# IvanPopov/video-flow-ml

Measured on AMD Instinct MI355X. Metric: flow-fields/sec @1080p seq5 MOF_sintel, higher is better.
Workload: dtype mixed (per-layer MFMA count, f32 accumulate): {"corr": 1, "update_block.encoder.convf1": 1, "update_block.encoder.convf2": 1, "update_block.gru.convq1.iter": "2a", "update_block.gru.convzr1.iter": 1, "update_block.gru.convzr2.iter": 1, "update_block.mask.0": 1, "update_block.mask.2": 1, "update_bloc

## Files before the change

### include/vfml.h

```cpp
#ifndef VFML_H
#define VFML_H
#include <stddef.h>
#include <stdint.h>

#ifdef __cplusplus
extern "C" {
#endif

#define VFML_ABI_VERSION 26

enum {
  VFML_EPI_NONE = 0,
  VFML_EPI_RELU = 1,
  VFML_EPI_TANH = 2,
  VFML_EPI_SIGMOID = 3,
  VFML_EPI_TANH_RELU = 4,
  VFML_EPI_GRU_ZR = 5,
  VFML_EPI_GRU_Q = 6,
  VFML_EPI_ADD_AUX = 7,
};

enum { VFML_FMT_F32 = 0, VFML_FMT_S16 = 1,
       VFML_FMT_F16 = 2 };

// ... 70 lines not shown
int vfml_instnorm_stats(const float* x, int n, int hw, int c, float eps,
                        float* stats, void* workspace, void* stream);
int vfml_instnorm_apply(const float* x, const float* stats, const float* res,
                        const float* res_stats, int n, int hw, int c, float* out, int out_fmt, void* stream);

int vfml_avgpool2x2(const float* x, int n, int h, int w, int c, float* out, void* stream);

int vfml_corr_lookup(const float* const* pyr, const int32_t* hl, const int32_t* wl,
                     const int32_t* ld, int levels, int radius, int nmaps, int q_per_map,
                     const float* coords, int ld_coords, float* out, int ld_out, int out_fmt, int vol_fmt, int vol_tile,
                     void* stream);
#define VFML_VOL_F16_LEVELS(m) (0x100 | (m))

int vfml_corr_lookup_indirect(const float* const* table, const int32_t* hl, const int32_t* wl, const int32_t* ld,
                              int levels, int radius, int nmaps, int q_per_map, const float* coords, int ld_coords,
                              float* out, int ld_out, int out_fmt, int vol_fmt, int vol_tile, void* stream);
int vfml_corr_lookup_indirect_bidir(const float* const* table, const int32_t* hl, const int32_t* wl, const int32_t* ld,
                                    int levels, int radius, int nmaps, int q_per_map, const float* coords, int ld_coords,
                                    int dir_coords, float* out, int ld_out, int dir_out, int dir_tab, int out_fmt, int vol_fmt,
                                    int vol_tile, void* stream);
int vfml_ptr_table_set(void* table, const void* const* ptrs, int n, void* stream);

#define VFML_SEED_NONE 0
#define VFML_SEED_LOAD 1
#define VFML_SEED_STORE 2
int vfml_window_seed(const void* cells, int ncentres, int rows, int cols, float* state, int ld_state, int h_off, int mf_off,
                     int ld_ctx, void* stream);

int vfml_flow_rows7(const float* flow, int n, int h, int w, float* rows, void* stream);

int vfml_conv3x3_c64(const float* in, int ld_in, int n, int h, int w, const void* w_hi, const void* w_lo, int kp, float w_scale,
                     const float* bias, float* out, int ldo, double* stats_part, void* stream);

int vfml_flow_half(const float* flow, int n, int h, int w, const void* w1_hi, int kp1, float w1_scale, const float* b1,
                   const void* w2_hi, int kp2, float w2_scale, const float* b2, float* out, int ld_out, void* stream);

int vfml_tapsum3x3(const float* t, int ld_t, const float* bias, int n, int h, int w, float* out, int parts, int64_t part_stride,
                   void* stream);
int vfml_tapsum3x3_update(const float* t, int ld_t, const float* bias, int n, int h, int w, int parts, int64_t part_stride,
                          float* coords1, float* flow_a, int ld_a, float* flow_b, int ld_b, int fmt_b, void* stream);

int vfml_coords_update(float* coords1, const float* delta, int n, int h, int w,
                       float* flow_a, int ld_a, float* flow_b, int ld_b, int fmt_b, void* stream);
int vfml_coords_init(float* coords1, int n, int h, int w, void* stream);

int vfml_convex_upsample(const float* coords1, int ch, const float* mask, int ld_mask,
                         int h, int w, float* out, void* stream);

int64_t vfml_instnorm_finalize_workspace_bytes(int chunks, int c);
int vfml_instnorm_finalize(const double* part, int n, int chunks, int c, int hw, float eps, float* stats,
                           void* workspace, int64_t workspace_bytes, void* stream);

int vfml_stem7x7s2_chunks(int h, int w);
int vfml_stem7x7s2(const float* frames, int n, int h, int w, const void* w_hi, const void* w_lo, float w_scale,
                   const float* bias, float* out, double* stats_part, void* stream);

int vfml_flow_lod(const float* flow, int h, int w, float* out, void* stream);

enum { VFML_ENCODE_GAMEDEV = 0, VFML_ENCODE_RG8 = 1, VFML_ENCODE_RGB8 = 2 };
int vfml_flow_encode(const float* flow, int h, int w, int mode, float width, float height, float scale,
                     float clamp, float two_clamp, unsigned char* out, void* stream);

enum { VFML_TAA_SIMPLE = 0, VFML_TAA_BILINEAR = 1, VFML_TAA_BILATERAL = 2 };
enum { VFML_PIX_U8 = 0, VFML_PIX_F32 = 1, VFML_PIX_F64 = 2 };
int vfml_taa_blend(const void* current, int cur_type, const float* flow, const void* history, int hist_type,
                   void* out, int out_type, int h, int w, int mode, double alpha, double sigma_color, void* stream);
// ... 102 lines not shown
```

### video-flow-ml_amd/vfml/hip.py

```python
import ctypes
import os
import subprocess
from ctypes import POINTER, c_char_p, c_double, c_float, c_int, c_int32, c_int64, c_void_p

import torch

_HERE = os.path.dirname(os.path.abspath(__file__))
LIB_PATH = os.environ.get("VFML_LIB") or os.path.join(_HERE, "libvfml_hip.so")
CSRC = os.path.join(_HERE, "csrc")
SOURCES = ["api.hip", "conv_gemm.hip", "conv_gemm_split.hip", "conv_gemm_tapx.hip", "conv_split_plan.hip", "stem.hip", "flow_half.hip", "enc_conv.hip", "norm_pool.hip", "flow_ops.hip", "effects.hip", "correct.hip", "render.hip", "text.hip", "turbulence.hip", "resize.hip", "jpeg.hip", "jpeg_decode.hip", "jpeg_decode_sync.hip", "deflate.hip", "attention.hip", "dwconv.hip"]

STATS_ROWS_F32, STATS_ROWS_S16 = 128, 32
EPI_NONE, EPI_RELU, EPI_TANH, EPI_SIGMOID, EPI_TANH_RELU, EPI_GRU_ZR, EPI_GRU_Q, EPI_ADD_AUX = range(8)
FMT_F32, FMT_S16, FMT_F16 = 0, 1, 2


def vol_f16_levels(mask):
    return 0x100 | mask


def _vol_mask(vol_fmt, levels):
    return (15 if vol_fmt == FMT_F16 else (vol_fmt & 15 if vol_fmt & 0x100 else 0)) & ((1 << levels) - 1)

KORDER_TAP, KORDER_CBLOCK, KORDER_CBLOCK64 = 0, 1, 2
CONV_SWAP_CROSS, CONV_MFMA2, CONV_MFMA1, CONV_MFMA2A, CONV_PER_TAP = 1, 2, 4, 8, 16


class ConvDesc(ctypes.Structure):
    _fields_ = [
        ("in0", c_void_p), ("c0", c_int32), ("ld0", c_int32),
        ("in1", c_void_p), ("c1", c_int32), ("ld1", c_int32),
        ("n", c_int32), ("h", c_int32), ("w", c_int32),
        ("weight", c_void_p), ("bias", c_void_p),
        ("cout", c_int32), ("kh", c_int32), ("kw", c_int32), ("stride", c_int32),
        ("pad_h", c_int32), ("pad_w", c_int32),
        ("out", c_void_p), ("ldo", c_int32),
        ("epilogue", c_int32), ("split", c_int32), ("out_scale", c_float),
        ("aux0", c_void_p), ("ld_aux0", c_int32),
        ("aux1", c_void_p), ("ld_aux1", c_int32),
        ("addend", c_void_p), ("ld_addend", c_int32),
        ("out_t", c_void_p), ("ld_out_t", c_int32),
        ("flags", c_int32),
        ("stats_part", c_void_p),
        ("ksplit_ws", c_void_p),
        ("proj_hi", c_void_p), ("proj_lo", c_void_p), ("proj_n", c_int32), ("proj_kp", c_int32), ("proj_scale", c_float),
        ("proj_out", c_void_p), ("ld_proj", c_int32),
        ("addend_ind", c_void_p),
    ]


COMMON_FLAGS = ["-fno-slp-vectorize"]
EXTRA_FLAGS = {}


def build(force=False, verbose=False):
    srcs = [os.path.join(CSRC, s) for s in SOURCES]
    hdrs = [os.path.join(CSRC, "vfml_common.h"), os.path.join(CSRC, "conv_split_common.h"),
# ... 54 lines not shown
    L.vfml_instnorm_workspace_bytes.argtypes = [c_int, c_int, c_int]
    L.vfml_instnorm_stats.argtypes = [c_void_p, c_int, c_int, c_int, c_float, c_void_p, c_void_p, c_void_p]
    L.vfml_softmax_rows_f16.argtypes = [c_void_p, c_int64, c_int, c_int64, c_void_p, c_int64, c_float, c_void_p]
    L.vfml_attention_plane_workspace_bytes.restype = c_int64
    L.vfml_attention_plane_workspace_bytes.argtypes = [c_int]
    L.vfml_attention_plane_f16.argtypes = [c_void_p, c_int64, c_void_p, c_int64, c_int, c_int, c_float, c_float, c_void_p, c_int64,
                                           c_void_p, c_void_p]
    L.vfml_dwconv2d.argtypes = [c_void_p, c_int64, c_int, c_int, c_int, c_int, c_int, c_void_p, c_void_p, c_void_p, c_int64, c_int, c_int,
                                c_int, c_void_p]
    L.vfml_gelu_rows.argtypes = [c_void_p, c_int64, c_void_p, c_int64, c_int64, c_int, c_int, c_int, c_void_p]
    L.vfml_transpose_to_s16.argtypes = [c_void_p, c_int, c_int, c_int, c_float, c_void_p, c_int64, c_void_p]
    L.vfml_add_to_s16.argtypes = [c_void_p, c_int64, c_void_p, c_int64, c_void_p, c_int64, c_int64, c_int, c_float, c_void_p]
    L.vfml_instnorm_finalize.argtypes = [c_void_p, c_int, c_int, c_int, c_int, c_float, c_void_p, c_void_p, c_int64, c_void_p]
    L.vfml_instnorm_finalize_workspace_bytes.restype = c_int64
    L.vfml_instnorm_finalize_workspace_bytes.argtypes = [c_int, c_int]
    L.vfml_stem7x7s2_chunks.argtypes = [c_int, c_int]
    L.vfml_stem7x7s2.argtypes = [c_void_p, c_int, c_int, c_int, c_void_p, c_void_p, c_float, c_void_p, c_void_p, c_void_p, c_void_p]
    L.vfml_instnorm_apply.argtypes = [c_void_p, c_void_p, c_void_p, c_void_p, c_int, c_int, c_int, c_void_p, c_int, c_void_p]
    L.vfml_avgpool2x2.argtypes = [c_void_p, c_int, c_int, c_int, c_int, c_void_p, c_void_p]
    L.vfml_corr_lookup.argtypes = [POINTER(c_void_p), POINTER(c_int32), POINTER(c_int32), POINTER(c_int32),
                                   c_int, c_int, c_int, c_int, c_void_p, c_int, c_void_p, c_int, c_int, c_int, c_int, c_void_p]
    L.vfml_corr_lookup_indirect.argtypes = [c_void_p, POINTER(c_int32), POINTER(c_int32), POINTER(c_int32),
                                            c_int, c_int, c_int, c_int, c_void_p, c_int, c_void_p, c_int, c_int, c_int, c_int,
                                            c_void_p]
    L.vfml_corr_lookup_indirect_bidir.argtypes = [c_void_p, POINTER(c_int32), POINTER(c_int32), POINTER(c_int32),
                                                  c_int, c_int, c_int, c_int, c_void_p, c_int, c_int, c_void_p, c_int, c_int,
                                                  c_int, c_int, c_int, c_int, c_void_p]
    L.vfml_ptr_table_set.argtypes = [c_void_p, POINTER(c_void_p), c_int, c_void_p]
    L.vfml_window_seed.argtypes = [c_void_p, c_int, c_int, c_int, c_void_p, c_int, c_int, c_int, c_int, c_void_p]
    L.vfml_tapsum3x3_update.argtypes = [c_void_p, c_int, c_void_p, c_int, c_int, c_int, c_int, ctypes.c_int64, c_void_p, c_void_p,
                                        c_int, c_void_p, c_int, c_int, c_void_p]
    L.vfml_conv3x3_c64.argtypes = [c_void_p, c_int, c_int, c_int, c_int, c_void_p, c_void_p, c_int, c_float, c_void_p, c_void_p,
                                   c_int, c_void_p, c_void_p]
    L.vfml_flow_half.argtypes = [c_void_p, c_int, c_int, c_int, c_void_p, c_int, c_float, c_void_p, c_void_p, c_int, c_float,
                                 c_void_p, c_void_p, c_int, c_void_p]
    L.vfml_coords_init.argtypes = [c_void_p, c_int, c_int, c_int, c_void_p]
    L.vfml_flow_rows7.argtypes = [c_void_p, c_int, c_int, c_int, c_void_p, c_void_p]
    L.vfml_tapsum3x3.argtypes = [c_void_p, c_int, c_void_p, c_int, c_int, c_int, c_void_p, c_int, ctypes.c_int64, c_void_p]
    L.vfml_coords_update.argtypes = [c_void_p, c_void_p, c_int, c_int, c_int, c_void_p, c_int, c_void_p, c_int,
                                     c_int, c_void_p]
    L.vfml_flow_lod.argtypes = [c_void_p, c_int, c_int, c_void_p, c_void_p]
    L.vfml_flow_encode.argtypes = [c_void_p, c_int, c_int, c_int, c_float, c_float, c_float, c_float, c_float, c_void_p,
                                   c_void_p]
    L.vfml_taa_blend.argtypes = [c_void_p, c_int, c_void_p, c_void_p, c_int, c_void_p, c_int, c_int, c_int, c_int, c_double,
                                 c_double, c_void_p]
    L.vfml_flow_quality_map.argtypes = [c_void_p, c_void_p, c_void_p, c_int, c_int, c_int, c_int, c_float, c_void_p, c_void_p]
    L.vfml_flow_correct_workspace_bytes.argtypes = [c_int, c_int]
    L.vfml_flow_correct_workspace_bytes.restype = ctypes.c_size_t
    L.vfml_flow_correct.argtypes = [c_void_p, c_void_p, c_void_p, c_void_p, c_int, c_int, c_int, c_int, c_void_p,
                                    c_double, c_double, c_double, c_double, c_double, c_void_p, c_void_p, c_void_p,
                                    ctypes.c_int64, c_void_p, ctypes.c_size_t, c_void_p]
    L.vfml_flow_colorize.argtypes = [c_void_p, c_int, c_int, c_int, c_void_p, c_void_p, c_void_p]
    L.vfml_flow_decode.argtypes = [c_void_p, c_int, c_int, c_int, c_float, c_void_p, c_void_p]
    L.vfml_flow_diff_overlay.argtypes = [c_void_p, c_void_p, c_int, c_int, c_void_p, c_void_p]
    L.vfml_compose_frame.argtypes = [POINTER(c_void_p), POINTER(c_int32), c_int, c_int, c_int, c_int, c_int64, c_void_p,
                                     c_void_p]
    L.vfml_text_draw.argtypes = [c_void_p, c_int, c_void_p, c_int, c_int, c_int64, c_int, c_void_p]
    L.vfml_flow_turbulence_workspace_bytes.argtypes = [c_int, c_int]
    L.vfml_flow_turbulence_workspace_bytes.restype = ctypes.c_size_t
    L.vfml_flow_turbulence_map.argtypes = [c_void_p, c_int, c_int, c_int, c_int, c_int, c_void_p, c_void_p, c_void_p, c_void_p,
                                           c_void_p, c_void_p]
    L.vfml_resize_u8.argtypes = [c_void_p, c_int, c_int, c_int, c_int64, c_void_p, c_int, c_int, c_int64, c_void_p, c_void_p,
                                 c_void_p]
    L.vfml_jpeg_workspace_bytes.restype = c_int64
    L.vfml_jpeg_workspace_bytes.argtypes = [c_int, c_int]
    L.vfml_jpeg_scan_capacity.restype = c_int64
# ... 12 lines not shown
                                       c_void_p, c_int64, c_void_p, c_void_p]
    L.vfml_jpeg_decode_sync_workspace_bytes.restype = c_int64
    L.vfml_jpeg_decode_sync_workspace_bytes.argtypes = [c_int, c_int, c_int64, c_int]
    L.vfml_jpeg_decode_rgb_sync.argtypes = [c_void_p, c_int64, c_int, c_int, c_int, c_void_p, c_void_p, c_int, c_int, c_int,
                                            c_void_p, c_void_p, c_int64, c_void_p, c_void_p]
    L.vfml_jpeg_decode_sampled_workspace_bytes.restype = c_int64
    L.vfml_jpeg_decode_sampled_workspace_bytes.argtypes = [c_int, c_int, c_int, c_int64]
    L.vfml_jpeg_decode_rgb_sampled.argtypes = [c_void_p, c_int64, c_int, c_int, c_int, c_int, c_void_p, c_void_p, c_int, c_int,
                                               c_void_p, c_void_p, c_int64, c_void_p, c_void_p]
    L.vfml_jpeg_decode_sync_sampled_workspace_bytes.restype = c_int64
    L.vfml_jpeg_decode_sync_sampled_workspace_bytes.argtypes = [c_int, c_int, c_int, c_int64, c_int]
    L.vfml_jpeg_decode_rgb_sync_sampled.argtypes = [c_void_p, c_int64, c_int, c_int, c_int, c_int, c_void_p, c_void_p, c_int,
                                                    c_int, c_int, c_void_p, c_void_p, c_int64, c_void_p, c_void_p]
    for fn in (L.vfml_deflate_capacity, L.vfml_deflate_workspace_bytes, L.vfml_inflate_workspace_bytes):
        fn.restype = c_int64
        fn.argtypes = [c_int64, c_int]
    L.vfml_deflate_huffman.argtypes = [c_void_p, c_int64, c_int, ctypes.c_uint32, c_void_p, c_void_p, c_int64, c_void_p, c_void_p,
                                       c_void_p, c_void_p]
    L.vfml_inflate_chunks.argtypes = [c_void_p, c_int64, c_void_p, c_int, c_int, c_int64, ctypes.c_uint32, c_void_p, c_void_p,
                                      c_void_p, c_void_p, c_void_p]
    L.vfml_convex_upsample.argtypes = [c_void_p, c_int, c_void_p, c_int, c_int, c_int, c_void_p, c_void_p]
    for name in EXPORTS:
        getattr(L, name)
    if L.vfml_abi_version() != 26:
        raise RuntimeError("libvfml_hip.so ABI version mismatch")
    _lib = L
    return L


EXPORTS = [
    "vfml_conv2d", "vfml_conv2d_split", "vfml_conv2d_variant", "vfml_conv2d_split_variant", "vfml_split_f16", "vfml_to_s16", "vfml_softmax_rows_s16", "vfml_softmax_rows_f16", "vfml_attention_plane_workspace_bytes", "vfml_attention_plane_f16", "vfml_dwconv2d", "vfml_gelu_rows", "vfml_transpose_to_s16", "vfml_add_to_s16",
    "vfml_transpose_split_f16", "vfml_frames_to_nhwc4", "vfml_instnorm_workspace_bytes", "vfml_instnorm_stats",
    "vfml_instnorm_apply", "vfml_instnorm_finalize", "vfml_instnorm_finalize_workspace_bytes", "vfml_avgpool2x2", "vfml_corr_lookup", "vfml_corr_lookup_indirect", "vfml_corr_lookup_indirect_bidir",
    "vfml_ptr_table_set", "vfml_window_seed", "vfml_coords_update", "vfml_coords_init", "vfml_tapsum3x3", "vfml_tapsum3x3_update", "vfml_flow_rows7", "vfml_flow_half", "vfml_conv3x3_c64",
    "vfml_convex_upsample", "vfml_stem7x7s2", "vfml_stem7x7s2_chunks", "vfml_flow_lod", "vfml_flow_encode", "vfml_taa_blend", "vfml_flow_quality_map", "vfml_flow_correct_workspace_bytes", "vfml_flow_correct",
    "vfml_flow_colorize", "vfml_compose_frame", "vfml_flow_decode", "vfml_flow_diff_overlay", "vfml_text_draw",
    "vfml_flow_turbulence_workspace_bytes", "vfml_flow_turbulence_map", "vfml_resize_u8",
    "vfml_jpeg_workspace_bytes", "vfml_jpeg_scan_capacity", "vfml_jpeg_encode_rgb",
    "vfml_jpeg_sampled_workspace_bytes", "vfml_jpeg_sampled_scan_capacity", "vfml_jpeg_encode_rgb_sampled",
    "vfml_jpeg_decode_workspace_bytes", "vfml_jpeg_decode_rgb",
    "vfml_jpeg_decode_sync_workspace_bytes", "vfml_jpeg_decode_rgb_sync",
    "vfml_jpeg_decode_sampled_workspace_bytes", "vfml_jpeg_decode_rgb_sampled",
    "vfml_jpeg_decode_sync_sampled_workspace_bytes", "vfml_jpeg_decode_rgb_sync_sampled",
    "vfml_deflate_capacity", "vfml_deflate_workspace_bytes", "vfml_deflate_huffman",
    "vfml_inflate_workspace_bytes", "vfml_inflate_chunks",
    "vfml_last_error", "vfml_abi_version",
]


def _check(rc, what):
    if rc != 0:
        raise RuntimeError(f"{what} failed (rc={rc}): {lib().vfml_last_error().decode()}")


def _stream():
    return c_void_p(torch.cuda.current_stream().cuda_stream)


def _ptr(t, offset=0):
    if t is None:
        return None
    return c_void_p(t.data_ptr() + 4 * offset)


def _dev(t, dtype=torch.float32):
    if not (t.is_cuda and t.dtype == dtype and t.is_contiguous()):
        raise ValueError(f"expected a contiguous {dtype} device tensor, got {t.dtype} {t.device} "
# ... 362 lines not shown
            x = torch.arange(w, device=dev, dtype=torch.int64).view(1, w)
            tpr = ((w - 1) >> self.tws) + 1
            pos = ((((y >> self.ths) * tpr + (x >> self.tws)) << (self.tws + self.ths))
                   + ((y & ((1 << self.ths) - 1)) << self.tws) + (x & ((1 << self.tws) - 1)))
            self._pos[key] = pos.reshape(-1).contiguous()
        return self._pos[key]

    def rows(self, x, h, w, c):
        n = self.count(h, w)
        out = torch.zeros(n, c, device=x.device, dtype=x.dtype)
        out.index_copy_(0, self.position(h, w, x.device), x.view(h * w, c))
        return out.view(-1)


def coords_init(coords1, n, h, w):
    _check(lib().vfml_coords_init(_ptr(_dev(coords1)), n, h, w, _stream()), "vfml_coords_init")


def flow_rows7(flow, n, h, w, rows):
    _check(lib().vfml_flow_rows7(_ptr(_dev(flow)), n, h, w, _ptr(_dev(rows)), _stream()), "vfml_flow_rows7")


def tapsum3x3(t, ld_t, bias, n, h, w, out, parts=1, part_stride=0):
    _check(lib().vfml_tapsum3x3(_ptr(_dev(t)), ld_t, _ptr(bias) if bias is not None else None, n, h, w, _ptr(_dev(out)),
                                parts, part_stride, _stream()), "vfml_tapsum3x3")


def conv3x3_c64(src, ld_in, n, h, w, weight, bias, out, ldo, stats_part=None, src_off=0):
    _check(lib().vfml_conv3x3_c64(_ptr(_dev(src), src_off), ld_in, n, h, w, c_void_p(weight.hi.data_ptr()),
                                  c_void_p(weight.lo.data_ptr()), weight.kp, weight.scale,
                                  _ptr(_dev(bias)) if bias is not None else None, _ptr(_dev(out)), ldo,
                                  c_void_p(stats_part.data_ptr()) if stats_part is not None else None, _stream()),
           "vfml_conv3x3_c64")


def flow_half(flow, n, h, w, w1, b1, w2, b2, out, ld_out, out_off=0):
    _check(lib().vfml_flow_half(_ptr(_dev(flow)), n, h, w, c_void_p(w1.hi.data_ptr()), w1.kp, w1.scale, _ptr(_dev(b1)),
                                c_void_p(w2.hi.data_ptr()), w2.kp, w2.scale, _ptr(_dev(b2)), _ptr(_dev(out), out_off), ld_out,
                                _stream()), "vfml_flow_half")


def tapsum3x3_update(t, ld_t, bias, n, h, w, coords1, parts=1, part_stride=0, flow_a=None, ld_a=0, flow_a_off=0, flow_b=None,
                     ld_b=0, flow_b_off=0, fmt_b=FMT_F32):
    _check(lib().vfml_tapsum3x3_update(_ptr(_dev(t)), ld_t, _ptr(bias) if bias is not None else None, n, h, w, parts, part_stride,
                                       _ptr(_dev(coords1)), _ptr(flow_a, flow_a_off), ld_a, _ptr(flow_b, flow_b_off), ld_b,
                                       fmt_b, _stream()), "vfml_tapsum3x3_update")


def coords_update(coords1, delta, n, h, w, flow_a=None, ld_a=0, flow_a_off=0, flow_b=None, ld_b=0, flow_b_off=0,
                  fmt_b=FMT_F32):
    _check(lib().vfml_coords_update(_ptr(_dev(coords1)), _ptr(delta), n, h, w,
                                    _ptr(flow_a, flow_a_off), ld_a, _ptr(flow_b, flow_b_off), ld_b, fmt_b, _stream()),
           "vfml_coords_update")


def flow_lods(flow, num_lods=5):
    lods = [_dev(flow.contiguous())]
    for _ in range(1, num_lods):
        h, w = lods[-1].shape[:2]
        out = torch.empty((h + 1) // 2, (w + 1) // 2, 2, device=flow.device, dtype=torch.float32)
        _check(lib().vfml_flow_lod(_ptr(lods[-1]), h, w, _ptr(out), _stream()), "vfml_flow_lod")
        lods.append(out)
    return lods


ENCODE_GAMEDEV, ENCODE_RG8, ENCODE_RGB8 = 0, 1, 2
# ... 573 lines not shown
```

### video-flow-ml_amd/vfml/network.py

```python
import os

import torch
import torch.nn as nn

from . import hip
from .weights import (BASE_CORR_LEVELS, BASE_CORR_RADIUS, GMA_NO_BIAS, conv_spec, corr_channel_subset, is_depthwise, pack_conv_weight,
                      pcblock_hidden, sk_blocks)

ATT_SCALE = 16384.0


def cor_pad(cor, split):
    return (cor + 15) // 16 * 16 if split else (cor + 3) // 4 * 4


def take_frames(src, idx):
    idx = list(idx)
    if all(b == a + 1 for a, b in zip(idx, idx[1:])):
        return src[idx[0]:idx[0] + len(idx)]
    return torch.stack([src[i] for i in idx])


class _Holder(nn.Module):

# ... 461 lines not shown
            s = st["next"]
            st["next"] = (s + 1) % st["R"]
            if s not in busy:
                break
        else:
            raise RuntimeError("attention store: every slot is in use by the current window")
        old = st["owner"][s]
        if old is not None and old != cache_key:
            self._feat_cache.pop(old, None)
        st["owner"][s] = cache_key
        return s

    def _build_attention(self, st, slot, cx, h8, w8, Pn, P, dev, AF):
        AD, ldA = self.ATT_DIM, st["ldA"]
        wgt, _ = P["att.to_qk"]
        nmq = self._nm("att.to_qk")
        if st["plain"]:
            qk = self._buf("att_qk", Pn * 2 * AD, dev)
            hip.conv2d(cx, 128, 256, 1, h8, w8, wgt, None, 2 * AD, 1, 1, qk, 2 * AD, in0_off=128, in_fmt=AF, mfma=nmq)
            hip.attention_plane(qk, qk, Pn, st["A"][slot], score_scale=1.0 / float(AD) ** 0.5, d=AD, ld_q=2 * AD, ld_k=2 * AD,
                                k_off=AD, workspace=self._buf("att_stats", 2 * Pn, dev))
            return
        qmap = self._buf("att_q", Pn * AD, dev)
        kmap = self._buf("att_k", Pn * AD, dev)
        hip.conv2d(cx, 128, 256, 1, h8, w8, wgt, None, AD, 1, 1, qmap, AD, in0_off=128, in_fmt=AF, out_fmt=AF, mfma=nmq)
        hip.conv2d(cx, 128, 256, 1, h8, w8, wgt, None, AD, 1, 1, kmap, AD, in0_off=128, weight_off=AD, in_fmt=AF, mfma=nmq)
        kw_ = st["k"].fill(kmap, scale=16.0)
        scores = self._buf("att_scores", Pn * ldA, dev)
        hip.conv2d(qmap, AD, AD, 1, 1, Pn, kw_, None, Pn, 1, 1, scores, ldA, out_scale=1.0 / float(AD) ** 0.5, in_fmt=AF)
        hip.softmax_rows_s16(scores, Pn, Pn, ldA, st["A"][slot], ldA, scale=ATT_SCALE)

    ITER0_RING = 8
    iter0_store = True

    def _iter0_store(self, dev, Pn, M):
        st = getattr(self, "_it0_store", None)
        if st is None or st["key"] != (str(dev), Pn) or st["ring"].R < M + 1:
            self._join_prefetch()
            for k in [k for k in self._feat_cache if k[0] == "m"]:
                del self._feat_cache[k]
            R = max(self.ITER0_RING, M + 1)
            st = self._it0_store = {"key": (str(dev), Pn), "ring": Iter0Ring(R, self._feat_cache),
                                    "S": torch.empty(R * Pn * 128, device=dev)}
        return st

    GRAPHS_KEPT = 8

    def _use_graph(self):
        use = getattr(self.cfg, "use_graph", None)
        if use is None:
            use = os.environ.get("VFML_GRAPH", "1") != "0"
        return bool(use) and hip._PROFILE is None

    def _run_body(self, body, key, dev):
        if not self._use_graph():
            body()
            return
        st = self._graphs.get(key)
        if st is None:
            body()
            while len(self._graphs) >= self.GRAPHS_KEPT:
                self._graphs.pop(next(iter(self._graphs)))
            self._graphs[key] = "seen"
            return
        if st == "seen":
            g = torch.cuda.CUDAGraph()
# ... 15 lines not shown
        def stats_of(t, hw, c, slot):
            s = st[slot * n * 128 * 2:]
            hip.instnorm_stats(t, n, hw, c, s, ws)
            return s

        split_prec = self._split()
        AF = hip.FMT_S16 if split_prec else hip.FMT_F32
        part_len = n * ((h2 * w2 + 31) // 32) * 64 * 2
        parts = self._buf("enc_part", 3 * part_len, dev, torch.float64) if split_prec else None
        fold_ws = self._buf("enc_foldws", min(n, 8) * 64 * 128 * 2, dev, torch.float64) if split_prec else None

        def conv_stats(src, c, hh_, ww_, name, planes, dst, slot, k, stride=1, pad=0, src_fmt=hip.FMT_F32):
            wgt, b = P[name]
            nm = self._nm(name) if split_prec else 3
            ho_, wo_ = (hh_ + 2 * pad - k) // stride + 1, (ww_ + 2 * pad - k) // stride + 1
            hw = ho_ * wo_
            rows = hip.STATS_ROWS_S16 if src_fmt == hip.FMT_S16 else hip.STATS_ROWS_F32
            if not (split_prec and (n == 1 or hw % rows == 0)):
                hip.conv2d(src, c, c, n, hh_, ww_, wgt, b, planes, k, k, dst, planes, stride=stride, pad_h=pad, pad_w=pad,
                           mfma=nm, in_fmt=src_fmt)
                return stats_of(dst, hw, planes, slot)
            chunks = (hw + rows - 1) // rows
            part = parts[slot * part_len:]
            if (c == 64 and planes == 64 and k == 3 and stride == 1 and pad == 1 and nm == 3 and src_fmt == hip.FMT_S16
                    and ww_ % 32 == 0 and getattr(wgt, "order", None) == hip.KORDER_CBLOCK and wgt.kp == 576 and wgt.lo is not None):
                hip.conv3x3_c64(src, c, n, hh_, ww_, wgt, b, dst, planes, stats_part=part)
            else:
                hip.conv2d(src, c, c, n, hh_, ww_, wgt, b, planes, k, k, dst, planes, stride=stride, pad_h=pad, pad_w=pad,
                           stats_part=part, mfma=nm, in_fmt=src_fmt)
            s = st[slot * n * 128 * 2:]
            hip.instnorm_finalize(part, n, chunks, planes, hw, s, workspace=fold_ws)
            return s

        stem = P.get(f"{prefix}.conv1.stem")
        if stem is not None and split_prec and self._nm(f"{prefix}.conv1") == 3:
            chunks = hip.stem_chunks(H, W)
            part = parts[0:]
            hip.stem7x7s2(x, n, H, W, stem[0], stem[1], raw, stats_part=part)
            s0 = st[0:]
            hip.instnorm_finalize(part, n, chunks, 64, h2 * w2, s0, workspace=fold_ws)
        else:
            s0 = conv_stats(x, 4, H, W, f"{prefix}.conv1", 64, raw, 0, 7, stride=2, pad=3)
        cur = act[0]
        hip.instnorm_apply(raw, s0, n, h2 * w2, 64, cur, out_fmt=AF)
        ch, hh, ww, ci = 64, h2, w2, 0
        for li, (planes, stride) in enumerate([(64, 1), (96, 2), (128, 2)], start=1):
            for bi in range(2):
                stv = stride if bi == 0 else 1
                ho, wo = (hh, ww) if stv == 1 else ((hh - 1) // 2 + 1, (ww - 1) // 2 + 1)
                name = f"{prefix}.layer{li}.{bi}"
                y = act[(ci + 1) % 3]
                nxt = act[(ci + 2) % 3]
                s1 = conv_stats(cur, ch, hh, ww, f"{name}.conv1", planes, raw, 0, 3, stride=stv, pad=1, src_fmt=AF)
                hip.instnorm_apply(raw, s1, n, ho * wo, planes, y, out_fmt=AF)
                s2 = conv_stats(y, planes, ho, wo, f"{name}.conv2", planes, raw, 1, 3, pad=1, src_fmt=AF)
                if stv != 1:
                    s3 = conv_stats(cur, ch, hh, ww, f"{name}.downsample.0", planes, raw2, 2, 1, stride=stv, src_fmt=AF)
                    hip.instnorm_apply(raw, s2, n, ho * wo, planes, nxt, res=raw2, res_stats=s3, out_fmt=AF)
                else:
                    hip.instnorm_apply(raw, s2, n, ho * wo, planes, nxt, res=cur, out_fmt=AF)
                cur, ci = nxt, (ci + 2) % 3
                ch, hh, ww = planes, ho, wo
        wgt, b = P[f"{prefix}.conv2"]
        hip.conv2d(cur, 128, 128, n, hh, ww, wgt, b, 256, 1, 1, out, ldo, out_off=out_off, epilogue=epilogue,
                   split=split, out_fmt=out_fmt, in_fmt=AF, mfma=self._nm(f"{prefix}.conv2") if split_prec else 3)
        return hh, ww

    @torch.no_grad()
    def forward(self, images, data=None, return_lowres=True):
        if not isinstance(images, torch.Tensor) or not images.is_cuda:
            raise RuntimeError("MOFNetHIP runs on an MI355X (HIP) device only; got "
                               f"{getattr(images, 'device', type(images))}. There is no CPU fallback in the shipped engine.")
        if images.dim() != 5 or images.shape[2] != 3:
            raise ValueError(f"images must be [B,N,3,H,W], got {tuple(images.shape)}")
        if images.shape[0] != 1:
            raise ValueError(f"Batch size must be 1, got {images.shape[0]}")
        src = images[0]
        if src.dtype != torch.float32:
            src = src.float()
        return self._run(src.contiguous(), src.shape[0], src.shape[2], src.shape[3], return_lowres)

    @torch.no_grad()
    def forward_u8(self, frames, return_lowres=True, frame_keys=None, tri_batch=False, pick_only=False):
        if not (isinstance(frames, torch.Tensor) and frames.is_cuda and frames.dtype == torch.uint8
                and frames.dim() == 4 and frames.shape[3] == 3):
            raise ValueError("forward_u8 expects a uint8 [N,H,W,3] device tensor")
        if frame_keys is not None and len(frame_keys) != frames.shape[0]:
            raise ValueError("frame_keys must have one entry per frame")
        if tri_batch and not self.tri_frame:
# ... 582 lines not shown
```

Baseline: 45.46.

## Fuse stride-2 conv1 and 1x1 downsample into one paired encoder kernel

Adds a dedicated HIP kernel that computes the 3x3 stride-2 conv1 and the 1x1 stride-2 downsample of the first layer2 block in a single pass. It shares the loaded input patch and reuses the centre-tap fragments for the 1x1 projection, and it fuses the instance-norm partial statistics for both outputs. This removes one full read of the input activation and separate launches for the two convs and their stats. The cost is a hand-tuned kernel that only handles 64->96 channels with split-precision weights, plus a fallback stats kernel when the output width is not a multiple of 32.

```diff
diff --git a/include/vfml.h b/include/vfml.h
--- a/include/vfml.h
+++ b/include/vfml.h
@@ -126,6 +126,11 @@
 int vfml_conv3x3_c64(const float* in, int ld_in, int n, int h, int w, const void* w_hi, const void* w_lo, int kp, float w_scale,
                      const float* bias, float* out, int ldo, double* stats_part, void* stream);
 
+int vfml_conv3x3s2_pair(const float* in, int cin, int ld_in, int in_fmt, int n, int h, int w, int cout,
+                        const void* w_hi, const void* w_lo, int kp, float w_scale, int k_order, const float* bias,
+                        const void* w2_hi, const void* w2_lo, int kp2, float w2_scale, int k_order2, const float* bias2,
+                        float* out, int ldo, double* stats_part, float* out2, int ldo2, double* stats_part2, void* stream);
+
 int vfml_flow_half(const float* flow, int n, int h, int w, const void* w1_hi, int kp1, float w1_scale, const float* b1,
                    const void* w2_hi, int kp2, float w2_scale, const float* b2, float* out, int ld_out, void* stream);
 
diff --git a/video-flow-ml_amd/vfml/csrc/enc_down.hip b/video-flow-ml_amd/vfml/csrc/enc_down.hip
--- /dev/null
+++ b/video-flow-ml_amd/vfml/csrc/enc_down.hip
@@ -0,0 +1,251 @@
+#include "conv_split_common.h"
+
+namespace {
+
+constexpr int ED_CIN = 64, ED_COUT = 96;
+constexpr int ED_NW = ED_COUT / 16, ED_NT = ED_NW * 64;
+constexpr int ED_TW = 32;
+constexpr int ED_PW = 2 * ED_TW + 1;
+constexpr int ED_HW = ED_TW + 1;
+constexpr int ED_PIX = 272;
+constexpr int ED_PATCH = 3 * 2 * ED_HW * ED_PIX;
+constexpr int ED_VLD = ED_COUT + 4;
+constexpr int ED_RES = ED_TW * ED_VLD;
+constexpr int ED_W2ROW = 2 * ED_CIN + 16;
+constexpr int ED_W2 = 2 * ED_COUT * ED_W2ROW;
+constexpr int ED_LDS = ED_PATCH + 2 * ED_RES * 4 + ED_W2;
+constexpr int ED_K = 9 * ED_CIN;
+constexpr int ED_NS = ED_K / 32;
+constexpr int ED_K2 = ED_CIN;
+constexpr int ED_NS2 = ED_K2 / 32;
+constexpr int ED_NPT = 9;
+static_assert(ED_NT == 24 * 16 && 3 * 24 >= ED_PW, "24 pixels x 16 pieces per pass, three passes cover a patch row");
+
+struct EncDownArgs {
+  const char* in;
+  const _Float16* whi; const _Float16* wlo;
+  const _Float16* w2hi; const _Float16* w2lo;
+  const float* bias; const float* bias2;
+  float* out; float* out2; int ldo, ldo2;
+  double* stats_part; double* stats_part2;
+  int ld_in, n, H, W, Ho, Wo, tiles_x;
+  int fused_stats;
+  float w_inv, w2_inv;
+};
+
+__global__ __launch_bounds__(ED_NT) void enc_down_pair_c64_kernel(const EncDownArgs a) {
+  extern __shared__ __attribute__((aligned(16))) char smem[];
+  float* sV = reinterpret_cast<float*>(smem + ED_PATCH);
+
+  const int t = threadIdx.x, lane = t & 63;
+  const int wave = __builtin_amdgcn_readfirstlane(t >> 6);
+  const int r4 = lane & 15, u4 = lane >> 4;
+  const int tiles_img = a.tiles_x * a.Ho;
+  const int total = a.n * tiles_img;
+
+  h16x8 bh[ED_NS], bl[ED_NS];
+  static_for<ED_NS>([&](auto sc) {
+    constexpr int s = decltype(sc)::value;
+    bh[s] = *reinterpret_cast<const h16x8*>(a.whi + (16 * wave + r4) * ED_K + s * 32 + u4 * 8);
+    bl[s] = *reinterpret_cast<const h16x8*>(a.wlo + (16 * wave + r4) * ED_K + s * 32 + u4 * 8);
+  });
+  char* sW2 = smem + ED_PATCH + 2 * ED_RES * 4;
+  for (int c = t; c < 2 * ED_COUT * 8; c += ED_NT) {
+    const int plane = c / (ED_COUT * 8), rem = c - plane * (ED_COUT * 8), row = rem >> 3, piece = rem & 7;
+    *reinterpret_cast<u32x4*>(sW2 + (plane * ED_COUT + row) * ED_W2ROW + piece * 16) =
+        *reinterpret_cast<const u32x4*>((plane ? a.w2lo : a.w2hi) + row * ED_K2 + piece * 8);
+  }
+  const char* w2l = sW2 + (16 * wave + r4) * ED_W2ROW + u4 * 16;
+  f32x4 bias4 = {0.f, 0.f, 0.f, 0.f}, bias4b = {0.f, 0.f, 0.f, 0.f};
+  if (a.bias) bias4 = *reinterpret_cast<const f32x4*>(a.bias + 16 * wave + 4 * u4);
+  if (a.bias2) bias4b = *reinterpret_cast<const f32x4*>(a.bias2 + 16 * wave + 4 * u4);
+
+  const int pcol = t >> 4;
+  char* pst = smem + ((pcol & 1) * ED_HW + (pcol >> 1)) * ED_PIX + (t & 15) * 16;
+  u32x4 pv[ED_NPT];
+  auto request = [&](int tile) {
+    const int img = tile / tiles_img, tl = tile - img * tiles_img;
+    const int oy = tl / a.tiles_x, tx = tl - oy * a.tiles_x;
+    const int iy0 = 2 * oy - 1, ix0 = 2 * (tx * ED_TW) - 1 + pcol;
+    const __amdgpu_buffer_rsrc_t rin = __builtin_amdgcn_make_buffer_rsrc(
+        const_cast<char*>(a.in) + (int64_t)img * a.H * a.W * a.ld_in * 4, 0, a.H * a.W * a.ld_in * 4, 0x00020000);
+    const int voff = ((iy0 * a.W + ix0) * a.ld_in) * 4 + (t & 15) * 16;
+    static_for<ED_NPT>([&](auto qc) {
+      constexpr int q = decltype(qc)::value, row = q / 3, k = q % 3;
+      const int iy = iy0 + row, ix = ix0 + 24 * k;
+      const bool ok = (unsigned)iy < (unsigned)a.H && (unsigned)ix < (unsigned)a.W && (k < 2 || pcol + 24 * k < ED_PW);
+      pv[q] = bload16(rin, ok ? voff + ((row * a.W + 24 * k) * a.ld_in) * 4 : (int)0x80000000);
+    });
+  };
+
+  int tile = blockIdx.x;
+  const int tile_end = total, tile_step = gridDim.x;
+  if (tile < tile_end) request(tile);
+  for (; tile < tile_end; tile += tile_step) {
+    const int img = tile / tiles_img, tl = tile - img * tiles_img;
+    const int oy = tl / a.tiles_x, tx = tl - oy * a.tiles_x;
+    const int ox0 = tx * ED_TW;
+
+    static_for<ED_NPT>([&](auto qc) {
+      constexpr int q = decltype(qc)::value, row = q / 3, k = q % 3;
+      if (k < 2 || pcol + 24 * k < ED_PW) *reinterpret_cast<u32x4*>(pst + (row * 2 * ED_HW + 12 * k) * ED_PIX) = pv[q];
+    });
+    lds_barrier();
+    if (tile + tile_step < tile_end) request(tile + tile_step);
+
+    f32x4 acc[2], acc2[2];
+#pragma unroll
+    for (int m = 0; m < 2; ++m) acc[m] = acc2[m] = f32x4{0.f, 0.f, 0.f, 0.f};
+    const char* al = smem + r4 * ED_PIX + u4 * 32;
+    h16x8 ah[2][2], alo[2][2];
+    auto frags = [&](auto sc) {
+      constexpr int s = decltype(sc)::value;
+      constexpr int cb = s / 9, ky = (s % 9) / 3, kx = s % 3;
+#pragma unroll
+      for (int m = 0; m < 2; ++m) {
+        const char* p = al + ((ky * 2 + (kx & 1)) * ED_HW + 16 * m + (kx >> 1)) * ED_PIX + cb * 128;
+        ah[s & 1][m] = *reinterpret_cast<const h16x8*>(p);
+        alo[s & 1][m] = *reinterpret_cast<const h16x8*>(p + 16);
+      }
+    };
+    frags(std::integral_constant<int, 0>{});
+    static_for<ED_NS>([&](auto sc) {
+      constexpr int s = decltype(sc)::value;
+      constexpr int cb = s / 9, ky = (s % 9) / 3, kx = s % 3, b = s & 1;
+      if constexpr (s + 1 < ED_NS) frags(std::integral_constant<int, s + 1>{});
+#pragma unroll
+      for (int m = 0; m < 2; ++m) acc[m] = __builtin_amdgcn_mfma_f32_16x16x32_f16(bh[s], ah[b][m], acc[m], 0, 0, 0);
+#pragma unroll
+      for (int m = 0; m < 2; ++m) acc[m] = __builtin_amdgcn_mfma_f32_16x16x32_f16(bl[s], ah[b][m], acc[m], 0, 0, 0);
+#pragma unroll
+      for (int m = 0; m < 2; ++m) acc[m] = __builtin_amdgcn_mfma_f32_16x16x32_f16(bh[s], alo[b][m], acc[m], 0, 0, 0);
+      if constexpr (ky == 1 && kx == 1) {
+        const h16x8 ch = *reinterpret_cast<const h16x8*>(w2l + cb * 64);
+        const h16x8 cl = *reinterpret_cast<const h16x8*>(w2l + ED_COUT * ED_W2ROW + cb * 64);
+#pragma unroll
+        for (int m = 0; m < 2; ++m) acc2[m] = __builtin_amdgcn_mfma_f32_16x16x32_f16(ch, ah[b][m], acc2[m], 0, 0, 0);
+#pragma unroll
+        for (int m = 0; m < 2; ++m) acc2[m] = __builtin_amdgcn_mfma_f32_16x16x32_f16(cl, ah[b][m], acc2[m], 0, 0, 0);
+#pragma unroll
+        for (int m = 0; m < 2; ++m) acc2[m] = __builtin_amdgcn_mfma_f32_16x16x32_f16(ch, alo[b][m], acc2[m], 0, 0, 0);
+      }
+      __builtin_amdgcn_sched_barrier(0);
+    });
+
+#pragma unroll
+    for (int m = 0; m < 2; ++m) {
+      f32x4 v, v2;
+#pragma unroll
+      for (int e = 0; e < 4; ++e) {
+        v[e] = acc[m][e] * a.w_inv + bias4[e];
+        v2[e] = acc2[m][e] * a.w2_inv + bias4b[e];
+      }
+      const int col = 16 * m + r4, ox = ox0 + col;
+      *reinterpret_cast<f32x4*>(&sV[col * ED_VLD + 16 * wave + 4 * u4]) = v;
+      *reinterpret_cast<f32x4*>(&sV[ED_RES + col * ED_VLD + 16 * wave + 4 * u4]) = v2;
+      if (ox < a.Wo) {
+        const int64_t px = ((int64_t)img * a.Ho + oy) * a.Wo + ox;
+        *reinterpret_cast<f32x4*>(a.out + px * a.ldo + 16 * wave + 4 * u4) = v;
+        *reinterpret_cast<f32x4*>(a.out2 + px * a.ldo2 + 16 * wave + 4 * u4) = v2;
+      }
+    }
+    lds_barrier();
+    if (a.fused_stats && t < 2 * ED_COUT) {
+      const int which = t >= ED_COUT ? 1 : 0, c = t - which * ED_COUT;
+      double* part = which ? a.stats_part2 : a.stats_part;
+      if (part) {
+        const float* col = sV + which * ED_RES + c;
+        double s1 = 0.0, s2 = 0.0;
+#pragma unroll 4
+        for (int x = 0; x < ED_TW; ++x) {
+          float f = col[x * ED_VLD], g;
+          asm("v_mov_b32 %0, %1" : "=v"(g) : "v"(f));
+          const double v = (double)g;
+          s1 += v;
+          s2 += v * v;
+        }
+        const int64_t chunk = ((((int64_t)img * a.Ho + oy) * a.Wo + ox0) >> 5);
+        double* o = part + (chunk * ED_COUT + c) * 2;
+        o[0] = s1;
+        o[1] = s2;
+      }
+    }
+  }
+}
+
+__global__ __launch_bounds__(256) void enc_down_stats_kernel(const float* __restrict__ out, int ldo, const float* __restrict__ out2,
+                                                             int ldo2, double* __restrict__ part, double* __restrict__ part2,
+                                                             int64_t M, int cout) {
+  const int64_t chunks = (M + 31) >> 5, jobs = chunks * 2 * cout;
+  for (int64_t j = (int64_t)blockIdx.x * blockDim.x + threadIdx.x; j < jobs; j += (int64_t)gridDim.x * blockDim.x) {
+    const int64_t chunk = j / (2 * cout);
+    const int rem = (int)(j - chunk * 2 * cout), which = rem >= cout ? 1 : 0, c = rem - which * cout;
+    double* o = which ? part2 : part;
+    if (!o) continue;
+    const float* src = which ? out2 : out;
+    const int ld = which ? ldo2 : ldo;
+    const int64_t p0 = chunk << 5, p1 = p0 + 32 < M ? p0 + 32 : M;
+    double s1 = 0.0, s2 = 0.0;
+    for (int64_t p = p0; p < p1; ++p) {
+      const double v = (double)src[p * ld + c];
+      s1 += v;
+      s2 += v * v;
+    }
+    o += (chunk * cout + c) * 2;
+    o[0] = s1;
+    o[1] = s2;
+  }
+}
+
+}
+
+extern "C" int vfml_conv3x3s2_pair(const float* in, int cin, int ld_in, int in_fmt, int n, int h, int w, int cout,
+                                   const void* w_hi, const void* w_lo, int kp, float w_scale, int k_order, const float* bias,
+                                   const void* w2_hi, const void* w2_lo, int kp2, float w2_scale, int k_order2, const float* bias2,
+                                   float* out, int ldo, double* stats_part, float* out2, int ldo2, double* stats_part2,
+                                   void* stream) {
+  VFML_REQUIRE(in && w_hi && w_lo && w2_hi && w2_lo && out && out2, "vfml_conv3x3s2_pair: null in / weight plane / out");
+  VFML_REQUIRE(n > 0 && h > 0 && w > 0, "vfml_conv3x3s2_pair: empty problem");
+  VFML_REQUIRE(cin == ED_CIN && cout == ED_COUT, "vfml_conv3x3s2_pair: built for 64 -> 96 channels (got %d -> %d)", cin, cout);
+  VFML_REQUIRE(in_fmt == VFML_FMT_S16, "vfml_conv3x3s2_pair: the input must be split rows (VFML_FMT_S16)");
+  VFML_REQUIRE(k_order == VFML_KORDER_CBLOCK && k_order2 == VFML_KORDER_CBLOCK,
+               "vfml_conv3x3s2_pair: both weights must be in VFML_KORDER_CBLOCK order");
+  VFML_REQUIRE(kp == ED_K && kp2 == ED_K2 && w_scale > 0.f && w2_scale > 0.f,
+               "vfml_conv3x3s2_pair: weight planes [%d][%d] and [%d][%d] with positive scales, got row pitches %d and %d", ED_COUT,
+               ED_K, ED_COUT, ED_K2, kp, kp2);
+  VFML_REQUIRE(ld_in >= cin && ld_in % 8 == 0 && ldo >= cout && ldo % 4 == 0 && ldo2 >= cout && ldo2 % 4 == 0,
+               "vfml_conv3x3s2_pair: ld_in >= %d (%% 8 == 0), ldo / ldo2 >= %d (%% 4 == 0); got %d, %d, %d", cin, cout, ld_in, ldo, ldo2);
+  VFML_REQUIRE((reinterpret_cast<uintptr_t>(in) & 31u) == 0 && vfml_aligned16(w_hi) && vfml_aligned16(w_lo) && vfml_aligned16(w2_hi) &&
+                   vfml_aligned16(w2_lo) && vfml_aligned16(bias) && vfml_aligned16(bias2) && vfml_aligned16(out) && vfml_aligned16(out2) &&
+                   (reinterpret_cast<uintptr_t>(stats_part) & 7u) == 0 && (reinterpret_cast<uintptr_t>(stats_part2) & 7u) == 0,
+               "vfml_conv3x3s2_pair: a 32-byte aligned split-row input, 16-byte aligned weights / biases / outputs, 8-byte "
+               "aligned stats_part");
+  const int ho = (h - 1) / 2 + 1, wo = (w - 1) / 2 + 1;
+  const int64_t hw_out = (int64_t)ho * wo;
+  VFML_REQUIRE(!(stats_part || stats_part2) || n == 1 || hw_out % VFML_STATS_ROWS_S16 == 0,
+               "vfml_conv3x3s2_pair: stats_part needs pixel blocks that do not straddle images (n == 1 or output pixels per "
+               "image %% %d == 0)", VFML_STATS_ROWS_S16);
+  EncDownArgs a;
+  a.in = reinterpret_cast<const char*>(in); a.ld_in = ld_in;
+  a.whi = reinterpret_cast<const _Float16*>(w_hi); a.wlo = reinterpret_cast<const _Float16*>(w_lo);
+  a.w2hi = reinterpret_cast<const _Float16*>(w2_hi); a.w2lo = reinterpret_cast<const _Float16*>(w2_lo);
+  a.bias = bias; a.bias2 = bias2;
+  a.out = out; a.out2 = out2; a.ldo = ldo; a.ldo2 = ldo2;
+  a.stats_part = stats_part; a.stats_part2 = stats_part2;
+  a.n = n; a.H = h; a.W = w; a.Ho = ho; a.Wo = wo; a.tiles_x = (wo + ED_TW - 1) / ED_TW;
+  a.fused_stats = (stats_part || stats_part2) && wo % ED_TW == 0;
+  a.w_inv = 1.0f / w_scale; a.w2_inv = 1.0f / w2_scale;
+  const int64_t total = (int64_t)n * a.tiles_x * ho;
+  VFML_REQUIRE(total < (1ll << 31) && (int64_t)h * w * ld_in * 4 < (1ll << 31) && (int64_t)n * hw_out < (1ll << 31),
+               "vfml_conv3x3s2_pair: an image of the input must stay below 2 GiB");
+  hipStream_t s = reinterpret_cast<hipStream_t>(stream);
+  if (const int rc = vfml_lds_cap(reinterpret_cast<const void*>(&enc_down_pair_c64_kernel), ED_LDS, "vfml_conv3x3s2_pair")) return rc;
+  const int grid = (int)(total < 256 ? total : 256);
+  hipLaunchKernelGGL(enc_down_pair_c64_kernel, dim3(grid), dim3(ED_NT), ED_LDS, s, a);
+  if ((stats_part || stats_part2) && !a.fused_stats) {
+    const int64_t M = (int64_t)n * hw_out, jobs = ((M + 31) >> 5) * 2 * cout;
+    const int g = (int)((jobs + 255) / 256 < 2048 ? (jobs + 255) / 256 : 2048);
+    hipLaunchKernelGGL(enc_down_stats_kernel, dim3(g), dim3(256), 0, s, out, ldo, out2, ldo2, stats_part, stats_part2, M, cout);
+  }
+  return vfml_check_launch("vfml_conv3x3s2_pair");
+}
diff --git a/video-flow-ml_amd/vfml/hip.py b/video-flow-ml_amd/vfml/hip.py
--- a/video-flow-ml_amd/vfml/hip.py
+++ b/video-flow-ml_amd/vfml/hip.py
@@ -8,7 +8,7 @@
 _HERE = os.path.dirname(os.path.abspath(__file__))
 LIB_PATH = os.environ.get("VFML_LIB") or os.path.join(_HERE, "libvfml_hip.so")
 CSRC = os.path.join(_HERE, "csrc")
-SOURCES = ["api.hip", "conv_gemm.hip", "conv_gemm_split.hip", "conv_gemm_tapx.hip", "conv_split_plan.hip", "stem.hip", "flow_half.hip", "enc_conv.hip", "norm_pool.hip", "flow_ops.hip", "effects.hip", "correct.hip", "render.hip", "text.hip", "turbulence.hip", "resize.hip", "jpeg.hip", "jpeg_decode.hip", "jpeg_decode_sync.hip", "deflate.hip", "attention.hip", "dwconv.hip"]
+SOURCES = ["api.hip", "conv_gemm.hip", "conv_gemm_split.hip", "conv_gemm_tapx.hip", "conv_split_plan.hip", "stem.hip", "flow_half.hip", "enc_conv.hip", "enc_down.hip", "norm_pool.hip", "flow_ops.hip", "effects.hip", "correct.hip", "render.hip", "text.hip", "turbulence.hip", "resize.hip", "jpeg.hip", "jpeg_decode.hip", "jpeg_decode_sync.hip", "deflate.hip", "attention.hip", "dwconv.hip"]
 
 STATS_ROWS_F32, STATS_ROWS_S16 = 128, 32
 EPI_NONE, EPI_RELU, EPI_TANH, EPI_SIGMOID, EPI_TANH_RELU, EPI_GRU_ZR, EPI_GRU_Q, EPI_ADD_AUX = range(8)
@@ -23,6 +23,7 @@
     return (15 if vol_fmt == FMT_F16 else (vol_fmt & 15 if vol_fmt & 0x100 else 0)) & ((1 << levels) - 1)
 
 KORDER_TAP, KORDER_CBLOCK, KORDER_CBLOCK64 = 0, 1, 2
+CONV3X3S2_PAIRS = ((64, 96),)
 CONV_SWAP_CROSS, CONV_MFMA2, CONV_MFMA1, CONV_MFMA2A, CONV_PER_TAP = 1, 2, 4, 8, 16
 
 
@@ -143,6 +144,10 @@
                                         c_int, c_void_p, c_int, c_int, c_void_p]
     L.vfml_conv3x3_c64.argtypes = [c_void_p, c_int, c_int, c_int, c_int, c_void_p, c_void_p, c_int, c_float, c_void_p, c_void_p,
                                    c_int, c_void_p, c_void_p]
+    L.vfml_conv3x3s2_pair.argtypes = [c_void_p, c_int, c_int, c_int, c_int, c_int, c_int, c_int,
+                                      c_void_p, c_void_p, c_int, c_float, c_int, c_void_p,
+                                      c_void_p, c_void_p, c_int, c_float, c_int, c_void_p,
+                                      c_void_p, c_int, c_void_p, c_void_p, c_int, c_void_p, c_void_p]
     L.vfml_flow_half.argtypes = [c_void_p, c_int, c_int, c_int, c_void_p, c_int, c_float, c_void_p, c_void_p, c_int, c_float,
                                  c_void_p, c_void_p, c_int, c_void_p]
     L.vfml_coords_init.argtypes = [c_void_p, c_int, c_int, c_int, c_void_p]
@@ -221,7 +226,7 @@
     "vfml_conv2d", "vfml_conv2d_split", "vfml_conv2d_variant", "vfml_conv2d_split_variant", "vfml_split_f16", "vfml_to_s16", "vfml_softmax_rows_s16", "vfml_softmax_rows_f16", "vfml_attention_plane_workspace_bytes", "vfml_attention_plane_f16", "vfml_dwconv2d", "vfml_gelu_rows", "vfml_transpose_to_s16", "vfml_add_to_s16",
     "vfml_transpose_split_f16", "vfml_frames_to_nhwc4", "vfml_instnorm_workspace_bytes", "vfml_instnorm_stats",
     "vfml_instnorm_apply", "vfml_instnorm_finalize", "vfml_instnorm_finalize_workspace_bytes", "vfml_avgpool2x2", "vfml_corr_lookup", "vfml_corr_lookup_indirect", "vfml_corr_lookup_indirect_bidir",
-    "vfml_ptr_table_set", "vfml_window_seed", "vfml_coords_update", "vfml_coords_init", "vfml_tapsum3x3", "vfml_tapsum3x3_update", "vfml_flow_rows7", "vfml_flow_half", "vfml_conv3x3_c64",
+    "vfml_ptr_table_set", "vfml_window_seed", "vfml_coords_update", "vfml_coords_init", "vfml_tapsum3x3", "vfml_tapsum3x3_update", "vfml_flow_rows7", "vfml_flow_half", "vfml_conv3x3_c64", "vfml_conv3x3s2_pair",
     "vfml_convex_upsample", "vfml_stem7x7s2", "vfml_stem7x7s2_chunks", "vfml_flow_lod", "vfml_flow_encode", "vfml_taa_blend", "vfml_flow_quality_map", "vfml_flow_correct_workspace_bytes", "vfml_flow_correct",
     "vfml_flow_colorize", "vfml_compose_frame", "vfml_flow_decode", "vfml_flow_diff_overlay", "vfml_text_draw",
     "vfml_flow_turbulence_workspace_bytes", "vfml_flow_turbulence_map", "vfml_resize_u8",
@@ -650,6 +655,20 @@
                                   _ptr(_dev(bias)) if bias is not None else None, _ptr(_dev(out)), ldo,
                                   c_void_p(stats_part.data_ptr()) if stats_part is not None else None, _stream()),
            "vfml_conv3x3_c64")
+
+
+def conv3x3s2_pair(src, c, ld_in, n, h, w, weight, bias, weight2, bias2, cout, out, ldo, out2, ldo2, stats_part=None,
+                    stats_part2=None, src_off=0, in_fmt=FMT_S16):
+    if weight.lo is None or weight2.lo is None:
+        raise ValueError("conv3x3s2_pair: SplitWeights with both planes")
+    _check(lib().vfml_conv3x3s2_pair(_ptr(_dev(src), src_off), c, ld_in, in_fmt, n, h, w, cout,
+                                     c_void_p(weight.hi.data_ptr()), c_void_p(weight.lo.data_ptr()), weight.kp, weight.scale,
+                                     weight.order, _ptr(_dev(bias)) if bias is not None else None,
+                                     c_void_p(weight2.hi.data_ptr()), c_void_p(weight2.lo.data_ptr()), weight2.kp, weight2.scale,
+                                     weight2.order, _ptr(_dev(bias2)) if bias2 is not None else None,
+                                     _ptr(_dev(out)), ldo, c_void_p(stats_part.data_ptr()) if stats_part is not None else None,
+                                     _ptr(_dev(out2)), ldo2, c_void_p(stats_part2.data_ptr()) if stats_part2 is not None else None,
+                                     _stream()), "vfml_conv3x3s2_pair")
 
 
 def flow_half(flow, n, h, w, w1, b1, w2, b2, out, ld_out, out_off=0):
diff --git a/video-flow-ml_amd/vfml/network.py b/video-flow-ml_amd/vfml/network.py
--- a/video-flow-ml_amd/vfml/network.py
+++ b/video-flow-ml_amd/vfml/network.py
@@ -517,6 +517,7 @@
 
     ITER0_RING = 8
     iter0_store = True
+    enc_down = True
 
     def _iter0_store(self, dev, Pn, M):
         st = getattr(self, "_it0_store", None)
@@ -598,6 +599,14 @@
             hip.instnorm_finalize(part, n, chunks, planes, hw, s, workspace=fold_ws)
             return s
 
+        def pair_ok(name1, name2, c, planes, hw):
+            if not (self.enc_down and split_prec and AF == hip.FMT_S16 and (c, planes) == (64, 96) and (n == 1 or hw % hip.STATS_ROWS_S16 == 0)):
+                return False
+            w1, w2 = P[name1][0], P[name2][0]
+            return (self._nm(name1) == 3 and self._nm(name2) == 3 and
+                    all(getattr(w_, "order", None) == hip.KORDER_CBLOCK and w_.lo is not None for w_ in (w1, w2)) and
+                    w1.kp == 9 * c and w2.kp == c)
+
         stem = P.get(f"{prefix}.conv1.stem")
         if stem is not None and split_prec and self._nm(f"{prefix}.conv1") == 3:
             chunks = hip.stem_chunks(H, W)
@@ -617,10 +626,22 @@
                 name = f"{prefix}.layer{li}.{bi}"
                 y = act[(ci + 1) % 3]
                 nxt = act[(ci + 2) % 3]
-                s1 = conv_stats(cur, ch, hh, ww, f"{name}.conv1", planes, raw, 0, 3, stride=stv, pad=1, src_fmt=AF)
+                paired = stv == 2 and pair_ok(f"{name}.conv1", f"{name}.downsample.0", ch, planes, ho * wo)
+                if paired:
+                    (wgt, b), (wgt2, b2) = P[f"{name}.conv1"], P[f"{name}.downsample.0"]
+                    hip.conv3x3s2_pair(cur, ch, ch, n, hh, ww, wgt, b, wgt2, b2, planes, raw, planes, raw2, planes,
+                                       stats_part=parts[0:], stats_part2=parts[2 * part_len:])
+                    s1 = st[0:]
+                    hip.instnorm_finalize(parts[0:], n, (ho * wo + 31) // 32, planes, ho * wo, s1, workspace=fold_ws)
+                else:
+                    s1 = conv_stats(cur, ch, hh, ww, f"{name}.conv1", planes, raw, 0, 3, stride=stv, pad=1, src_fmt=AF)
                 hip.instnorm_apply(raw, s1, n, ho * wo, planes, y, out_fmt=AF)
                 s2 = conv_stats(y, planes, ho, wo, f"{name}.conv2", planes, raw, 1, 3, pad=1, src_fmt=AF)
-                if stv != 1:
+                if paired:
+                    s3 = st[2 * n * 128 * 2:]
+                    hip.instnorm_finalize(parts[2 * part_len:], n, (ho * wo + 31) // 32, planes, ho * wo, s3, workspace=fold_ws)
+                    hip.instnorm_apply(raw, s2, n, ho * wo, planes, nxt, res=raw2, res_stats=s3, out_fmt=AF)
+                elif stv != 1:
                     s3 = conv_stats(cur, ch, hh, ww, f"{name}.downsample.0", planes, raw2, 2, 1, stride=stv, src_fmt=AF)
                     hip.instnorm_apply(raw, s2, n, ho * wo, planes, nxt, res=raw2, res_stats=s3, out_fmt=AF)
                 else:
```

After: 45.61 (median of 6 runs). About the same (+0.3%).
